# xmlyqing00/V-FloodNet

Hardware: AMD Instinct MI355X
Metric: segmented frames/sec at 480p (higher is better)
Workload: dtype f32

## Files before the change

include/vfn_hip.h:

```cpp
#ifndef VFN_HIP_H
#define VFN_HIP_H

#ifdef __cplusplus
extern "C" {
#endif

#define VFN_ABI_VERSION 15
enum { VFN_DESC_CONV = 0, VFN_DESC_STEM = 1, VFN_DESC_BANKSCAN = 2, VFN_DESC_MEMREAD = 3, VFN_DESC_BANK = 4, VFN_DESC_WGRAD = 5,
       VFN_DESC_REFRESH_FILTER = 6, VFN_DESC_REFRESH_EPILOGUE = 7, VFN_DESC_GATHER = 8, VFN_DESC_BANKMATCH = 9 };
int vfn_abi_version(void);
int vfn_sizeof_desc(int which);

typedef struct vfn_conv_desc {
    const float* in;
    const float* w;
    const float* scale;
    const float* shift;
    const float* res;
    float* out;
    int N, H, W, Cin, in_ld;
    int Ho, Wo, Cout, cout_pad, out_ld, res_ld;
    int KH, KW, stride, pad;
    int relu_in, relu_out;
    int M;
    int ksplit;
    int split_from;
    int res_mod;
    float* partial;
    int* tile_counters;
    int w_packed;
    int in_lp;
    int out_lp_relu;
    void* out_lp;
    const float* mask;
    int mask_ld;
    int mask_after;
    int w_batch_rows;
    int k_rot;
} vfn_conv_desc;

int vfn_conv_cfg_count(void);
int vfn_conv_cfg_tile(int cfg, int* bm, int* bn);
int vfn_conv_cfg_info(int cfg, int* bm, int* bn, int* wm, int* wn, int* dma);
int vfn_conv_cfg_modes(int cfg);
int vfn_conv_cfg_wk(int cfg);
int vfn_conv_cfg_tpb(int cfg);
#define VFN_CONV_SK_WS_FLOATS (16 * 1024 * 1024)
#define VFN_CONV_SK_MAX_TILES 16384
int vfn_conv_cfg_kind(int cfg);
int vfn_conv_cfg_name(int cfg, char* buf, int n);
int vfn_conv2d_nhwc_f32(const vfn_conv_desc* d, int cfg, void* stream);
int vfn_conv2d_nhwc_bf16(const vfn_conv_desc* d, int cfg, void* stream);
int vfn_conv2d_nhwc_bf16x3(const vfn_conv_desc* d, int cfg, void* stream);

int vfn_winograd_tiles(int N, int H, int W);
int vfn_winograd_input_f32(const float* x, int N, int H, int W, int C, int ld_x, int relu, float* V, int rows_pad, void* stream);
int vfn_winograd_output_f32(const float* Mb, int rows_pad, int N, int H, int W, int Cout, const float* scale, const float* shift,
                            const float* res, int res_ld, int res_mod, int relu_out, float* out, int out_ld, void* stream);
int vfn_winograd_output_masked_f32(const float* Mb, int rows_pad, int N, int H, int W, int Cout, const float* res, int res_ld,
                                   const float* mask, int mask_ld, int mask_after, float* out, int out_ld, void* stream);
int vfn_winograd_gemm_f32(const float* V, const float* U, float* Mb, int comps, int rows_pad, int C, int Cout, int cout_pad, int cfg,
                          int wgs, void* stream);
int vfn_conv1x1_persistent_f32(const vfn_conv_desc* d, int cfg, int wgs, void* stream);
int vfn_winograd_input_bf16(const float* x, int N, int H, int W, int C, int ld_x, int relu, void* V, int rows_pad, void* stream);
int vfn_winograd_gemm_bf16(const void* V, const void* U, float* Mb, int comps, int rows_pad, int C, int Cout, int cout_pad, int cfg,
                           int wgs, void* stream);
int vfn_winograd_gy_f32(const float* gy, int N, int H, int W, int C, int ld, float* Z, int rows_pad, void* stream);
int vfn_winograd_dw_f32(const float* dU, int Cout, int Cin, const float* rowscale, float* dw, int accumulate, void* stream);

typedef struct vfn_stem_desc {
    const float* frame;
    const float* mask;
    const float* w;
    const float* scale;
    const float* shift;
    float* out;
    float mean[3];
    float std[3];
    int N, cin;
    int H0, W0;
    int pad_top, pad_left;
    int Hp, Wp;
    int Ho, Wo;
} vfn_stem_desc;

int vfn_stem_conv7x7_f32(const vfn_stem_desc* d, void* stream);
int vfn_maxpool3x3s2_nhwc_f32(const float* in, float* out, int N, int H, int W, int C, void* stream);

int vfn_upsample2x_add_nhwc_f32(const float* s, const float* pm, float* out, int N, int h, int w, int C,
                                int s_bcast, void* stream);
// ... 85 lines not shown
int vfn_softmax_cols_backward_f32(const float* P, const float* dP, int B, int Q, int ld, float scale, float* dS, void* stream);
int vfn_adamw_f32(float* p, const float* g, float* m, float* v, long long n, double lr, double beta1, double beta2, double eps,
                  double weight_decay, int step, void* stream);
int vfn_colsum_f32(const float* x, int M, int C, int ld, float* partial, int nb, float* out, void* stream);
#define VFN_COLSUM_COUNTERS 64
int vfn_colsum_acc_f32(const float* x, int M, int C, int ld, float* partial, int nb, float* out, int accumulate, int* counter,
                       void* stream);
int vfn_upsample2x_add_backward_f32(const float* gm, float* gs, float* gpm, int N, int h, int w, int C, int s_bcast,
                                    void* stream);
int vfn_segment_loss_f32(const float* logit, const int* label, int bs, int obj_n, int n, float lu, float* partial, float* stats,
                         float* grad, void* stream);
int vfn_segment_uncertainty_backward_f32(const float* logit, int bs, int obj_n, int n, const float* g_unc_dev,
                                         const float* g_scores, float* partial, float* stats, float* grad, void* stream);
int vfn_tail_grad_o_f32(const float* G, const float* p_up, const float* unc, const float* conf, const float* q, float* g_o,
                        int obj_n, int h, int w, int pad_top, int pad_left, int H0, int W0, void* stream);
int vfn_tail_split_f32(const float* g_p2, const float* unc, const float* conf, const float* q, float* g_q, float* g_cf, float* g_u,
                       int obj_n, int npix, void* stream);
int vfn_local_stats_backward_f32(const float* g_lm, const float* lm, const float* g_cf, const float* g_u, const float* g_p2,
                                 const float* r1, const float* rough, const float* p_up, float* dA, float* dBv, int* amax,
                                 float* g_r1, float* g_pup, int obj_n, int h, int w, int C, void* stream);

typedef struct vfn_bankscan_desc {
    const float* q;
    const float* bank_k;
    const int* bank_len;
    const float* rowscale;
    float* part;
    long long stride_q, stride_k, stride_rs;
    float scale;
    int ldq, q_per_obj, HW, obj_n, nsplit, mode;
    int precision;
    int* work_counter;
    const void* bank_k_lp;
    float* scores;
    long long stride_scores;
} vfn_bankscan_desc;

typedef struct vfn_memread_desc {
    const float* q;
    const float* qv;
    const float* bank_k;
    const float* bank_v;
    const int* bank_len;
    const float* ml;
    float* o_part;
    int* cnt;
    float* info;
    float* out;
    long long stride_k, stride_v, stride_cnt, stride_info;
    float scale, thres;
    int ldq, ldqv, ld_out, HW, obj_n, nsplit;
    int precision;
    const void* bank_k_lp;
    const void* bank_v_lp;
    const float* scores;
    long long stride_scores;
} vfn_memread_desc;

int vfn_bank_scan(const vfn_bankscan_desc* d, void* stream);
int vfn_bank_scan_finish(const float* part, int nsplit, int HW, int obj_n, int mode, float* ml, int* idx,
                         float* corr, const float* colscale, void* stream);
int vfn_memread_apply(const vfn_memread_desc* d, void* stream);

typedef struct vfn_bankmatch_desc {
    const float* q;
    const float* bank_k;
    const void* bank_k_lp;
    const int* bank_len;
    const float* rowscale;
    const float* qnorm;
    const float* colscale;
    float* part_x3;
    float* part_f32;
    int* ulist;
    int* ucount;
    int* utotal;
    int* work_counter;
    int* match_idx;
    float* match_corr;
    long long stride_q, stride_k, stride_rs;
    int ldq, HW, obj_n;
    int nsplit;
    int nsplit_fb;
} vfn_bankmatch_desc;
int vfn_bank_match_certified(const vfn_bankmatch_desc* d, void* stream);
int vfn_memread_finish(const vfn_memread_desc* d, void* stream);

#define VFN_BANK_MAX_HW 32768
typedef struct vfn_bank_desc {
    float* bank_k;
    float* bank_v;
    float* info;
    float* scratch_k;
    float* scratch_v;
    float* scratch_info;
    const int* bank_len;
    int* bank_len_rw;
    const float* bank_knorm;
    const float* bank_vnorm;
    const int* match_idx;
    const float* match_corr;
    const float* new_k;
    const float* new_knorm;
    const float* new_vnorm;
    int* app_pos;
    int* keep_dst;
    int* plan;
    int* stats;
    long long stride_k, stride_v, stride_info, stride_n, stride_new;
    double class_budget;
    float thres_close, update_rate, new_hit_init;
    int frame_idx, ld_new, voff, HW, obj_n, cap;
    int rm_class;
    int rm_request;
} vfn_bank_desc;

int vfn_bank_refresh_lp(const vfn_bank_desc* d, void* bank_k_lp, void* bank_v_lp, int all_rows, void* stream);
int vfn_bank_refresh_lp_keys(const vfn_bank_desc* d, void* bank_k_lp, int all_rows, void* stream);

int vfn_row_norms(const float* x, long long stride_obj, int ld, int dim, const int* len_dev, int rows,
                  int obj_n, float* nrm, float* inv , long long stride_n, void* stream);
int vfn_bank_merge(const vfn_bank_desc* d, void* stream);
int vfn_bank_append(const vfn_bank_desc* d, void* stream);
int vfn_bank_remove(const vfn_bank_desc* d, void* stream);
int vfn_bank_refresh_norms(const vfn_bank_desc* d, float* bank_knorm, float* bank_kinv, float* bank_vnorm, void* stream);
int vfn_scatter_mean_f32(const float* src, long long src_s0, long long src_s1, const long long* index,
                         int S, float* out, long long out_s0, long long out_s1, int D, void* stream);
int vfn_scatter_mean_checked_f32(const float* src, long long src_s0, long long src_s1, const long long* index,
                                 long long index_s0, int S, float* out, long long out_s0, long long out_s1, int D,
                                 long long B, int* status, void* stream);

int vfn_resize_bicubic_f32(const float* in, float* out, int C, int Hi, int Wi, int Ho, int Wo, void* stream);
int vfn_resize_nearest_f32(const float* in, float* out, int C, int Hi, int Wi, int Ho, int Wo, void* stream);
int vfn_softmax_objects_f32(const float* score, float* prob, int obj_n, int n, void* stream);
int vfn_resize_argmax_u8(const float* prob, unsigned char* label, int obj_n, int Hi, int Wi, int Ho, int Wo,
                         void* stream);
int vfn_postprocess_pred_u8(const unsigned char* pred_host, int H, int W, unsigned char* out_host);
int vfn_postprocess_pred_device_u8(const unsigned char* pred, unsigned char* out, int* scratch, int H, int W,
                                   void* stream);

int vfn_to_tensor_u8(const unsigned char* src, float* dst, int H, int W, void* stream);
int vfn_overlay_u8(const float* frame, const unsigned char* mask, const unsigned char* palette, int* scratch,
                   unsigned char* out, int H, int W, double alpha, double cscale, void* stream);

int vfn_jpeg_entropy_decode(const unsigned char* data, long long size, short* coef, long long coef_cap,
                            unsigned short* qt, int* info);
int vfn_jpeg_idct_u8(const short* coef, const unsigned short* qt, unsigned char* plane, int blocks_per_row,
                     int block_rows, int pitch, void* stream);
int vfn_jpeg_to_tensor_f32(const unsigned char* y, const unsigned char* cb, const unsigned char* cr, int pitch_y,
                           int pitch_c, int W, int H, int hs, int vs, int ncomp, float* out_f32, unsigned char* out_u8,
                           void* stream);

int vfn_png_sizes(int H, int W, int bpp, long long* work_bytes, long long* out_bytes);
int vfn_png_deflate_u8(const unsigned char* raw, int H, int W, int bpp, void* work, unsigned char* out, int* stats,
                       void* stream);

int vfn_png_unfilter_sizes(int width, int height, int bpp, int* pitch, long long* work_bytes);
int vfn_png_unfilter_u8(const unsigned char* filtered, int width, int height, int bpp, void* work, unsigned char* raw,
                        int* status, void* stream);
int vfn_png_to_tensor_f32(const unsigned char* raw, int pitch, int width, int height, int color_type,
                          const unsigned char* palette, float* out, unsigned char* out_u8, void* stream);

int vfn_ln_stem_f32(const float* x, const float* w, const float* scale, const float* shift, float* out, int N, int H, int W, int Ho,
                    int Wo, int ld, int pad_before, void* stream);
int vfn_ln_dwconv_f32(const float* x, const float* w, const float* scale, const float* shift, float* out, int N, int H, int W, int C,
                      int ld_x, int ld_out, int k, int stride, int pad_before, int Ho, int Wo, int swish_in, void* stream);
// ... 20 lines not shown
```

v-floodnet_amd/_lib.py:

```python
import ctypes as C
import os

import torch

_HERE = os.path.dirname(os.path.abspath(__file__))
LIB_PATH = os.environ.get('VFN_LIB_PATH') or os.path.join(_HERE, 'libvfn_hip.so')

_lib = None

c_fp = C.c_void_p


class ConvDesc(C.Structure):
    _fields_ = [('inp', c_fp), ('w', c_fp), ('scale', c_fp), ('shift', c_fp), ('res', c_fp), ('out', c_fp),
                ('N', C.c_int), ('H', C.c_int), ('W', C.c_int), ('Cin', C.c_int), ('in_ld', C.c_int),
                ('Ho', C.c_int), ('Wo', C.c_int), ('Cout', C.c_int), ('cout_pad', C.c_int),
                ('out_ld', C.c_int), ('res_ld', C.c_int),
                ('KH', C.c_int), ('KW', C.c_int), ('stride', C.c_int), ('pad', C.c_int),
                ('relu_in', C.c_int), ('relu_out', C.c_int), ('M', C.c_int), ('ksplit', C.c_int),
                ('split_from', C.c_int), ('res_mod', C.c_int), ('partial', c_fp), ('tile_counters', c_fp),
                ('w_packed', C.c_int), ('in_lp', C.c_int), ('out_lp_relu', C.c_int), ('out_lp', c_fp), ('mask', c_fp), ('mask_ld', C.c_int), ('mask_after', C.c_int), ('w_batch_rows', C.c_int), ('k_rot', C.c_int)]


class WgradDesc(C.Structure):
    _fields_ = [('x', c_fp), ('gy', c_fp), ('rowscale', c_fp), ('dw', c_fp), ('partial', c_fp),
                ('N', C.c_int), ('H', C.c_int), ('W', C.c_int), ('Cin', C.c_int), ('ld_x', C.c_int),
                ('Ho', C.c_int), ('Wo', C.c_int), ('Cout', C.c_int), ('ld_g', C.c_int),
                ('k', C.c_int), ('stride', C.c_int), ('pad', C.c_int), ('relu', C.c_int), ('accumulate', C.c_int), ('ksplit', C.c_int),
                ('tile_counters', c_fp), ('batch', C.c_int), ('reserved', C.c_int), ('x_bstride', C.c_longlong), ('g_bstride', C.c_longlong)]


class RefreshFilter(C.Structure):
    _fields_ = [('src', c_fp), ('dst', c_fp), ('gamma', c_fp), ('var', c_fp), ('eps', C.c_float), ('kind', C.c_int),
                ('cout', C.c_int), ('cin', C.c_int), ('cin_off', C.c_int), ('cin_total', C.c_int), ('kh', C.c_int), ('kw', C.c_int),
                ('dst_ld', C.c_int), ('dst_row0', C.c_int), ('dst_col0', C.c_int), ('cout_ld', C.c_int), ('block0', C.c_int),
                ('reserved', C.c_int)]


class RefreshEpilogue(C.Structure):
    _fields_ = [('gamma', c_fp), ('beta', c_fp), ('mean', c_fp), ('var', c_fp), ('scale', c_fp), ('shift', c_fp),
                ('eps', C.c_float), ('C', C.c_int)]


class GatherEntry(C.Structure):
    _fields_ = [('src', c_fp), ('dst_offset', C.c_longlong), ('stride', C.c_longlong * 4), ('shape', C.c_int * 4), ('block0', C.c_int),
                ('reserved', C.c_int)]


class StemDesc(C.Structure):
    _fields_ = [('frame', c_fp), ('mask', c_fp), ('w', c_fp), ('scale', c_fp), ('shift', c_fp), ('out', c_fp),
                ('mean', C.c_float * 3), ('std', C.c_float * 3),
                ('N', C.c_int), ('cin', C.c_int), ('H0', C.c_int), ('W0', C.c_int),
                ('pad_top', C.c_int), ('pad_left', C.c_int), ('Hp', C.c_int), ('Wp', C.c_int),
                ('Ho', C.c_int), ('Wo', C.c_int)]


class BankScanDesc(C.Structure):
    _fields_ = [('q', c_fp), ('bank_k', c_fp), ('bank_len', c_fp), ('rowscale', c_fp), ('part', c_fp),
                ('stride_q', C.c_longlong), ('stride_k', C.c_longlong), ('stride_rs', C.c_longlong),
                ('scale', C.c_float),
                ('ldq', C.c_int), ('q_per_obj', C.c_int), ('HW', C.c_int), ('obj_n', C.c_int),
                ('nsplit', C.c_int), ('mode', C.c_int), ('precision', C.c_int), ('work_counter', c_fp), ('bank_k_lp', c_fp), ('scores', c_fp), ('stride_scores', C.c_longlong)]


class MemReadDesc(C.Structure):
    _fields_ = [('q', c_fp), ('qv', c_fp), ('bank_k', c_fp), ('bank_v', c_fp), ('bank_len', c_fp), ('ml', c_fp),
                ('o_part', c_fp), ('cnt', c_fp), ('info', c_fp), ('out', c_fp),
                ('stride_k', C.c_longlong), ('stride_v', C.c_longlong), ('stride_cnt', C.c_longlong),
                ('stride_info', C.c_longlong),
                ('scale', C.c_float), ('thres', C.c_float),
                ('ldq', C.c_int), ('ldqv', C.c_int), ('ld_out', C.c_int), ('HW', C.c_int), ('obj_n', C.c_int),
                ('nsplit', C.c_int), ('precision', C.c_int), ('bank_k_lp', c_fp), ('bank_v_lp', c_fp), ('scores', c_fp), ('stride_scores', C.c_longlong)]


class BankMatchDesc(C.Structure):
    _fields_ = [('q', c_fp), ('bank_k', c_fp), ('bank_k_lp', c_fp), ('bank_len', c_fp), ('rowscale', c_fp), ('qnorm', c_fp),
                ('colscale', c_fp), ('part_x3', c_fp), ('part_f32', c_fp), ('ulist', c_fp), ('ucount', c_fp), ('utotal', c_fp),
                ('work_counter', c_fp), ('match_idx', c_fp), ('match_corr', c_fp),
                ('stride_q', C.c_longlong), ('stride_k', C.c_longlong), ('stride_rs', C.c_longlong),
                ('ldq', C.c_int), ('HW', C.c_int), ('obj_n', C.c_int), ('nsplit', C.c_int), ('nsplit_fb', C.c_int)]


class BankDesc(C.Structure):
    _fields_ = [('bank_k', c_fp), ('bank_v', c_fp), ('info', c_fp),
                ('scratch_k', c_fp), ('scratch_v', c_fp), ('scratch_info', c_fp),
                ('bank_len', c_fp), ('bank_len_rw', c_fp), ('bank_knorm', c_fp), ('bank_vnorm', c_fp),
                ('match_idx', c_fp), ('match_corr', c_fp), ('new_k', c_fp), ('new_knorm', c_fp), ('new_vnorm', c_fp),
                ('app_pos', c_fp), ('keep_dst', c_fp), ('plan', c_fp), ('stats', c_fp),
                ('stride_k', C.c_longlong), ('stride_v', C.c_longlong), ('stride_info', C.c_longlong),
                ('stride_n', C.c_longlong), ('stride_new', C.c_longlong),
                ('class_budget', C.c_double),
                ('thres_close', C.c_float), ('update_rate', C.c_float), ('new_hit_init', C.c_float),
                ('frame_idx', C.c_int), ('ld_new', C.c_int), ('voff', C.c_int), ('HW', C.c_int),
                ('obj_n', C.c_int), ('cap', C.c_int), ('rm_class', C.c_int), ('rm_request', C.c_int)]


ABI_VERSION = 15
DESC_IDS = {0: ConvDesc, 1: StemDesc, 2: BankScanDesc, 3: MemReadDesc, 4: BankDesc, 5: WgradDesc, 6: RefreshFilter, 7: RefreshEpilogue, 8: GatherEntry, 9: BankMatchDesc}


def lib():
    global _lib
    if _lib is None:
        if not os.path.isfile(LIB_PATH):
            raise RuntimeError(
                f'{LIB_PATH} not found: build the HIP kernels first '
                '(python -c "import __graft_entry__ as g; g.build()" or make -C v-floodnet_amd/csrc)')
        L = C.CDLL(LIB_PATH)
        L.vfn_abi_version.restype = C.c_int
        if L.vfn_abi_version() != ABI_VERSION:
            raise RuntimeError(f'{LIB_PATH} has ABI version {L.vfn_abi_version()}, this package expects {ABI_VERSION} '
                               '(descriptor layouts differ): rebuild it (make -C v-floodnet_amd/csrc)')
        L.vfn_sizeof_desc.restype = C.c_int
        for which, cls in DESC_IDS.items():
            if L.vfn_sizeof_desc(which) != C.sizeof(cls):
                raise RuntimeError(f'{LIB_PATH}: sizeof({cls.__name__}) is {L.vfn_sizeof_desc(which)} in the library, '
                                   f'{C.sizeof(cls)} in this binding: rebuild it (make -C v-floodnet_amd/csrc)')
        _declare(L)
        _lib = L
    return _lib


def _declare(L):
    i, f, p = C.c_int, C.c_float, C.c_void_p
    L.vfn_abi_version.restype = i
    L.vfn_conv_cfg_count.restype = i
    L.vfn_conv_cfg_tile.argtypes = [i, C.POINTER(i), C.POINTER(i)]
    L.vfn_conv_cfg_info.argtypes = [i] + [C.POINTER(i)] * 5
    L.vfn_conv_cfg_wk.argtypes = [i]
    L.vfn_conv_cfg_wk.restype = i
    L.vfn_conv_cfg_tpb.argtypes = [i]
    L.vfn_conv_cfg_tpb.restype = i
    L.vfn_conv_cfg_modes.argtypes = [i]
    L.vfn_conv_cfg_modes.restype = i
    L.vfn_conv_cfg_kind.argtypes = [i]
    L.vfn_conv_cfg_name.argtypes = [i, C.c_char_p, i]
    L.vfn_conv_cfg_name.restype = i
    L.vfn_conv_cfg_kind.restype = i
    L.vfn_sizeof_desc.argtypes = [i]
    L.vfn_conv2d_nhwc_f32.argtypes = [C.POINTER(ConvDesc), i, p]
    L.vfn_conv2d_nhwc_bf16.argtypes = [C.POINTER(ConvDesc), i, p]
    L.vfn_conv2d_nhwc_bf16x3.argtypes = [C.POINTER(ConvDesc), i, p]
    L.vfn_stem_conv7x7_f32.argtypes = [C.POINTER(StemDesc), p]
    L.vfn_bank_scan.argtypes = [C.POINTER(BankScanDesc), p]
    L.vfn_memread_apply.argtypes = [C.POINTER(MemReadDesc), p]
    L.vfn_memread_finish.argtypes = [C.POINTER(MemReadDesc), p]
    L.vfn_bank_merge.argtypes = [C.POINTER(BankDesc), p]
    L.vfn_bank_append.argtypes = [C.POINTER(BankDesc), p]
    L.vfn_bank_remove.argtypes = [C.POINTER(BankDesc), p]
    L.vfn_bank_refresh_norms.argtypes = [C.POINTER(BankDesc), p, p, p, p]
    L.vfn_conv_wgrad_f32.argtypes = [C.POINTER(WgradDesc), p]
    L.vfn_bank_refresh_lp.argtypes = [C.POINTER(BankDesc), p, p, i, p]
    L.vfn_bank_refresh_lp_keys.argtypes = [C.POINTER(BankDesc), p, i, p]
    L.vfn_bank_match_certified.argtypes = [C.POINTER(BankMatchDesc), p]
    L.vfn_stem_wgrad_scratch_floats.argtypes = [i]
    L.vfn_stem_wgrad_scratch_floats.restype = i
    for name, args in SIGNATURES.items():
        fn = getattr(L, name)
        fn.argtypes = args
        fn.restype = i


_i, _f, _p = C.c_int, C.c_float, C.c_void_p
_ll = C.c_longlong
SIGNATURES = {
    'vfn_maxpool3x3s2_nhwc_f32': [_p, _p, _i, _i, _i, _i, _p],
    'vfn_upsample2x_add_nhwc_f32': [_p, _p, _p, _i, _i, _i, _i, _i, _p],
    'vfn_upsample2x_add_lp_nhwc_f32': [_p, _p, _p, _p, _i, _i, _i, _i, _i, _i, _p],
    'vfn_rough_uncertainty_f32': [_p, _p, _p, _p, _i, _i, _i, _p],
    'vfn_transpose_taps_f32': [_p, _i, _i, _i, _i, _i, _i, _i, _i, _i, _i, _i, _p, _p, _i, _p],
    'vfn_dilate2_f32': [_p, _p, _i, _i, _i, _i, _i, _i, _p],
    'vfn_bn_param_grads_f32': [_p, _p, _p, _p, _p, _i, _i, _p, _i, _p, _p, _p],
    'vfn_bn_param_grads_acc_f32': [_p, _p, _p, _p, _p, _i, _i, _p, _i, _p, _p, _i, _p, _p],
    'vfn_maxpool3x3s2_backward_f32': [_p, _p, _p, _i, _i, _i, _i, _p, _i, _p],
    'vfn_softmax_cols_f32': [_p, _i, _i, _i, _f, _p, _p],
    'vfn_softmax_cols_backward_f32': [_p, _p, _i, _i, _i, _f, _p, _p],
    'vfn_adamw_f32': [_p, _p, _p, _p, _ll, C.c_double, C.c_double, C.c_double, C.c_double, C.c_double, _i, _p],
    'vfn_colsum_f32': [_p, _i, _i, _i, _p, _i, _p, _p],
    'vfn_colsum_acc_f32': [_p, _i, _i, _i, _p, _i, _p, _i, _p, _p],
    'vfn_upsample2x_add_backward_f32': [_p, _p, _p, _i, _i, _i, _i, _i, _p],
# ... 125 lines not shown
```

v-floodnet_amd/csrc/memory_read.hip:

```cpp
#include "common.h"
#include "../../include/vfn_hip.h"
#include <type_traits>
#include <cstdlib>

namespace {

constexpr int DK = 128, DV = 512;
constexpr int CH = 64;

__device__ __forceinline__ int swz(int row, int chunk) { return row * DK + ((chunk ^ (row & 15)) << 2); }

__device__ __forceinline__ int swz64(int row, int chunk) { return row * CH + ((chunk ^ (row & 15)) << 2); }

__device__ __forceinline__ void chunk_load_async(float* sK, const float* src, int valid, int wave, int lane) {
#pragma unroll
    for (int j = 0; j < 8; ++j) {
        const int r = (wave * 8 + j) * 2 + (lane >> 5);
        const int pc = lane & 31;
        const int rr = min(r, valid - 1);
        const float* g = src + (size_t)rr * DK + ((pc ^ (r & 15)) << 2);
        __builtin_amdgcn_global_load_lds(g, sK + (wave * 8 + j) * 2 * DK, 16, 0, 0);
    }
}

__device__ __forceinline__ void score_tile(const float* sK, const float* sQ, int wr, int wq, int li, int lh, f32x16& acc) {
#pragma unroll
    for (int r = 0; r < 16; ++r) acc[r] = 0.f;
    const int ra = wr * 32 + li, rq = wq * 32 + li;
    f32x4 a[2], b[2];
    a[0] = *reinterpret_cast<const f32x4*>(sK + swz(ra, lh));
    b[0] = *reinterpret_cast<const f32x4*>(sQ + swz(rq, lh));
#pragma unroll
    for (int kk = 0; kk < 16; ++kk) {
        const int cur = kk & 1;
        if (kk + 1 < 16) {
            a[cur ^ 1] = *reinterpret_cast<const f32x4*>(sK + swz(ra, 2 * (kk + 1) + lh));
            b[cur ^ 1] = *reinterpret_cast<const f32x4*>(sQ + swz(rq, 2 * (kk + 1) + lh));
        }
#pragma unroll
        for (int t = 0; t < 4; ++t)
            acc = __builtin_amdgcn_mfma_f32_32x32x2f32(a[cur][t], b[cur][t], acc, 0, 0, 0);
    }
}

typedef __attribute__((ext_vector_type(2))) float f32x2;
typedef unsigned u32x4 __attribute__((ext_vector_type(4)));
typedef unsigned u32x2 __attribute__((ext_vector_type(2)));
typedef __attribute__((ext_vector_type(4))) __bf16 bf16x4;
typedef __attribute__((ext_vector_type(8))) __bf16 bf16x8;

__device__ __forceinline__ bf16x8 cvt8(const f32x4& a, const f32x4& b) {
    bf16x8 r;
#pragma unroll
    for (int e = 0; e < 4; ++e) { r[e] = (__bf16)a[e]; r[4 + e] = (__bf16)b[e]; }
    return r;
}
__device__ __forceinline__ void split8(const f32x4& a, const f32x4& b, bf16x8& h, bf16x8& l) {
#pragma unroll
    for (int e = 0; e < 4; ++e) {
        const __bf16 x = (__bf16)a[e], y = (__bf16)b[e];
        h[e] = x; h[4 + e] = y;
        l[e] = (__bf16)(a[e] - (float)x); l[4 + e] = (__bf16)(b[e] - (float)y);
    }
}
__device__ __forceinline__ int swzk(int row, int half, int chunk) { return row * 512 + half * 256 + ((chunk ^ (row & 15)) << 4); }
__device__ __forceinline__ int swzq(int row, int chunk) { return row * 256 + ((chunk ^ (row & 15)) << 4); }
__device__ __forceinline__ int swzp(int row, int chunk) { return row * 128 + ((chunk ^ ((row >> 1) & 7)) << 4); }

template <int NT, bool X3>
__device__ __forceinline__ void convert_chunk_inplace(float* sK, int tid) {
    constexpr int TPR = NT / CH;
    constexpr int F4 = 32 / TPR;
    const int r = tid / TPR, part = tid % TPR;
    f32x4 v[F4];
#pragma unroll
    for (int j = 0; j < F4; ++j) v[j] = *reinterpret_cast<const f32x4*>(sK + swz(r, part * F4 + j));
    __syncthreads();
    char* base = reinterpret_cast<char*>(sK);
#pragma unroll
    for (int j = 0; j < F4; j += 2) {
        bf16x8 h, l;
        split8(v[j], v[j + 1], h, l);
        const int chunk = (part * F4 + j) >> 1;
        *reinterpret_cast<bf16x8*>(base + swzk(r, 0, chunk)) = h;
// ... 439 lines not shown
#pragma unroll
                    for (int j = 0; j < 4; ++j) {
                        const int row = row0 + j;
                        if (row < B) {
                            const float s_ = acc[i][4 * g + j] * sc[j];
                            if (s_ > run_m) { run_m = s_; run_i = row; }
                        }
                    }
                }
        }
        if (c + 1 < c_hi) store_k(PAR ^ 1, std::integral_constant<int, PAR ^ 1>{});
        __syncthreads();
    };
    for (int c = c_lo; c < c_hi; c += 2) {
        body(std::integral_constant<int, 0>{}, c);
        if (c + 1 < c_hi) body(std::integral_constant<int, 1>{}, c + 1);
    }

    {
        const float om = __shfl_xor(run_m, 32, 64);
        if (MODE == 0) {
            const float ol = __shfl_xor(run_l, 32, 64);
            const float mn = fmaxf(run_m, om);
            float l = 0.f;
            if (mn > -INFINITY) l = run_l * expf(run_m - mn) + ol * expf(om - mn);
            run_m = mn; run_l = l;
        } else {
            const int oi = __shfl_xor(run_i, 32, 64);
            if (om > run_m || (om == run_m && oi < run_i)) { run_m = om; run_i = oi; }
        }
    }
    const int q = q0 + li;
    if (lh == 0 && q < p.HW) {
        float* dst = p.part + (((size_t)obj * p.nsplit + split) * p.HW + q) * 2;
        dst[0] = run_m;
        dst[1] = (MODE == 0) ? run_l : __int_as_float(run_i);
    }
  }
}

template <int MODE>
__global__ void bank_scan_finish_kernel(const float* __restrict__ part, int nsplit, int HW, int obj_n,
                                        float* __restrict__ ml, int* __restrict__ idx, float* __restrict__ corr,
                                        const float* __restrict__ colscale) {
    const int t = blockIdx.x * blockDim.x + threadIdx.x;
    const int i = min(t >> 3, obj_n * HW - 1), j = t & 7;
    const bool live = (t >> 3) < obj_n * HW;
    const int obj = i / HW, q = i - obj * HW;
    float m = -INFINITY, x = (MODE == 0) ? 0.f : __int_as_float(0x7fffffff);
    auto fold = [&](float om, float ox) {
        if (MODE == 0) {
            const float mn = fmaxf(m, om);
            if (mn > -INFINITY) x = x * expf(m - mn) + ox * expf(om - mn);
            m = mn;
        } else {
            const int i0 = __float_as_int(x), i1 = __float_as_int(ox);
            if (om > m || (om == m && i1 < i0)) { m = om; x = ox; }
        }
    };
    for (int s = j; s < nsplit; s += 8) {
        const float* src = part + (((size_t)obj * nsplit + s) * HW + q) * 2;
        fold(src[0], src[1]);
    }
    const int base = (threadIdx.x & 63) & ~7;
#pragma unroll
    for (int o = 1; o < 8; ++o) {
        const float om = __shfl(m, base + o, 64), ox = __shfl(x, base + o, 64);
        if (j == 0) fold(om, ox);
    }
    if (j != 0 || !live) return;
    if (MODE == 0) { ml[(size_t)i * 2] = m; ml[(size_t)i * 2 + 1] = x; }
    else { idx[i] = __float_as_int(x); corr[i] = m * colscale[i]; }
}

constexpr float MATCH_EPS_REL = 1.25e-4f;
constexpr float MATCH_EPS_ABS = 5.421010862427522e-20f;
constexpr float MATCH_QNORM_MAX = 1.152921504606846976e18f;

__global__ __launch_bounds__(64)
void bank_match_certify_kernel(const vfn_bankmatch_desc p) {
    const int lane = threadIdx.x, li = lane & 31, lh = lane >> 5;
    const int obj = blockIdx.y, q0 = blockIdx.x * 32;
    const int q = q0 + li, qc = min(q, p.HW - 1);
    float m = -INFINITY, m2 = -INFINITY;
    int bi = 0x7fffffff;
    auto fold = [&](float om, int oi, float o2) {
        if (om > m || (om == m && oi < bi)) { m2 = fmaxf(fmaxf(m, m2), o2); m = om; bi = oi; }
        else m2 = fmaxf(fmaxf(m2, om), o2);
    };
    const float* part = p.part_x3 + ((size_t)obj * p.nsplit * p.HW + qc) * 4;
#pragma unroll 4
    for (int s = lh; s < p.nsplit; s += 2) {
        const f32x4 v = *reinterpret_cast<const f32x4*>(part + (size_t)s * p.HW * 4);
        fold(v[0], __float_as_int(v[1]), v[2]);
    }
    fold(__shfl_xor(m, 32, 64), __shfl_xor(bi, 32, 64), __shfl_xor(m2, 32, 64));

    const size_t col = (size_t)obj * p.HW + qc;
    const float qn = p.qnorm[col];
    const float margin = 4.f * (MATCH_EPS_REL * qn + MATCH_EPS_ABS);
    const bool cert = q < p.HW && qn > 0.f && qn <= MATCH_QNORM_MAX && m > -INFINITY && m < INFINITY && (m - m2) > margin;

    const float* krow = p.bank_k + (size_t)obj * p.stride_k + (size_t)(cert ? bi : 0) * DK + 4 * lh;
    const float* qrow = p.q + (size_t)obj * p.stride_q + (size_t)qc * p.ldq + 4 * lh;
    f32x16 acc;
#pragma unroll
    for (int r = 0; r < 16; ++r) acc[r] = 0.f;
#pragma unroll
    for (int kk = 0; kk < 16; ++kk) {
        f32x4 a = *reinterpret_cast<const f32x4*>(krow + 8 * kk);
        const f32x4 b = *reinterpret_cast<const f32x4*>(qrow + 8 * kk);
        if (!cert) a = f32x4{0.f, 0.f, 0.f, 0.f};
#pragma unroll
        for (int t = 0; t < 4; ++t) acc = __builtin_amdgcn_mfma_f32_32x32x2f32(a[t], b[t], acc, 0, 0, 0);
    }
    const int rsel = (li & 3) + 4 * (li >> 3);
    float dot = 0.f;
#pragma unroll
    for (int r = 0; r < 16; ++r) dot = (r == rsel) ? acc[r] : dot;
    if (lh != ((li >> 2) & 1)) return;
    if (cert) {
        const float s_ = dot * p.rowscale[(size_t)obj * p.stride_rs + bi];
        p.match_idx[col] = bi;
        p.match_corr[col] = s_ * p.colscale[col];
    } else if (q < p.HW) {
        const int pos = atomicAdd(p.ucount + obj, 1);
        p.ulist[(size_t)obj * p.HW + pos] = q;
        if (p.utotal) atomicAdd(p.utotal + obj, 1);
    }
}

__global__ void bank_match_finish_listed_kernel(const float* __restrict__ part, int nsplit, int HW, int obj_n,
                                                const int* __restrict__ ulist, const int* __restrict__ ucount,
                                                int* __restrict__ idx, float* __restrict__ corr, const float* __restrict__ colscale) {
    const int t = blockIdx.x * blockDim.x + threadIdx.x;
    const int i = min(t >> 3, obj_n * HW - 1), j = t & 7;
    const int obj = i / HW, pos = i - obj * HW;
    const bool live = (t >> 3) < obj_n * HW && pos < ucount[obj];
    float m = -INFINITY, x = __int_as_float(0x7fffffff);
    auto fold = [&](float om, float ox) {
        const int i0 = __float_as_int(x), i1 = __float_as_int(ox);
        if (om > m || (om == m && i1 < i0)) { m = om; x = ox; }
    };
    if (live)
        for (int s = j; s < nsplit; s += 8) {
            const float* src = part + (((size_t)obj * nsplit + s) * HW + pos) * 2;
            fold(src[0], src[1]);
        }
    const int base = (threadIdx.x & 63) & ~7;
#pragma unroll
    for (int o = 1; o < 8; ++o) {
        const float om = __shfl(m, base + o, 64), ox = __shfl(x, base + o, 64);
        if (j == 0) fold(om, ox);
    }
    if (j != 0 || !live) return;
    const size_t c = (size_t)obj * HW + ulist[(size_t)obj * HW + pos];
    idx[c] = __float_as_int(x);
    corr[c] = m * colscale[c];
}

__device__ __forceinline__ int softmax_hits(f32x16& acc, float scale, float qm, float qinv, float thres, int nvalid, int rloc) {
    int cnt = 0;
#ifdef VFN_ABLATE_SOFTMAX
    for (int r = 0; r < 16; ++r) acc[r] *= qinv;
    return cnt;
#endif
    const float sm = -qm;
    if (nvalid >= CH) {
#pragma unroll
        for (int r = 0; r < 16; ++r) acc[r] = fast_exp(fmaf(acc[r], scale, sm)) * qinv;
    } else {
#pragma unroll
        for (int r = 0; r < 16; ++r) {
            const int rr = rloc + (r & 3) + 8 * (r >> 2);
            const float pv = fast_exp(fmaf(acc[r], scale, sm)) * qinv;
            acc[r] = rr < nvalid ? pv : 0.f;
        }
    }
#pragma unroll
    for (int r = 0; r < 16; ++r) {
        const unsigned long long hit = __ballot(acc[r] > thres);
        const int rlo = (r & 3) + 8 * (r >> 2);
        const int c_lo = __popcll(hit & 0xffffffffull), c_hi = __popcll(hit >> 32);
        asm volatile("v_writelane_b32 %0, %1, %2" : "+v"(cnt) : "s"(c_lo), "n"(rlo));
        asm volatile("v_writelane_b32 %0, %1, %2" : "+v"(cnt) : "s"(c_hi), "n"(rlo + 4));
    }
    return cnt;
}

__device__ int vfn_apply_linear_order = 0;
__device__ __forceinline__ void apply_item(const vfn_memread_desc& p, int& split, int& qt, int& obj) {
    const int qtiles = (int)gridDim.x / p.nsplit;
    if (vfn_apply_linear_order) { split = blockIdx.x % p.nsplit; qt = blockIdx.x / p.nsplit; obj = blockIdx.y; return; }
    const int total = (int)(gridDim.x * gridDim.y);
    const int id = (int)(blockIdx.y * gridDim.x + blockIdx.x);
    const int q = total >> 3, r = total & 7;
    const int xcd = id & 7, slot = id >> 3;
    const int L = (xcd < r ? xcd * (q + 1) : r * (q + 1) + (xcd - r) * q) + slot;
    const int pair = L / qtiles;
    qt = L - pair * qtiles;
    obj = pair / p.nsplit;
    split = pair - obj * p.nsplit;
}

constexpr int QTW = 128;
__device__ __forceinline__ void apply_slice(const vfn_memread_desc& p, int& split, int& qt, int& obj, int& q0, int& B) {
    apply_item(p, split, qt, obj);
// ... 1017 lines not shown
```

v-floodnet_amd/feature_bank.py:

```python
import numpy as np
import torch

from . import _lib, ops
from ._lib import ptr, stream, check, BankDesc, BankScanDesc, BankMatchDesc

DK, DV = 128, 512
MAX_SPLIT = 20
MAX_SPLIT_SCAN = 256
QT, QT_SCAN, CH = 64, 128, 64
MAX_HW = 32768


def pick_scan_slices(hw, obj_n, b_upper, target_items=1536, min_chunks=8):
    nchunks = max(1, (b_upper + CH - 1) // CH)
    qtiles = (hw + QT_SCAN - 1) // QT_SCAN
    import os
    if os.environ.get('VFN_NSPLIT_SCAN'):
        return max(1, min(int(os.environ['VFN_NSPLIT_SCAN']), nchunks, MAX_SPLIT_SCAN))
    want = max(1, target_items // (qtiles * obj_n))
    return max(1, min(want, nchunks // min_chunks if nchunks >= min_chunks else 1, MAX_SPLIT_SCAN))


def pick_fallback_slices(obj_n, b_upper, target_items=512, min_chunks=4):
    nchunks = max(1, (b_upper + CH - 1) // CH)
# ... 57 lines not shown
        _lib.lib()

    def _alloc(self, hw, n_init):
        self._require_gpu()
        dev = self.device
        o = self.obj_n
        cap = (int(max(self.class_budget, n_init)) + 2 * hw + 2 * CH + 63) // 64 * 64
        self._cap, self._hw = cap, hw
        self._kbuf = torch.empty(o, cap, DK, device=dev)
        self._vbuf = torch.empty(o, cap, DV, device=dev)
        self._ibuf = torch.zeros(o, cap, 2, device=dev)
        self._len_dev = torch.zeros(o, dtype=torch.int32, device=dev)
        self._stats = torch.zeros(o, 4, dtype=torch.int32, device=dev)
        self._knorm = torch.empty(o, cap, device=dev)
        self._vnorm = torch.empty(o, cap, device=dev)
        self._kinv = torch.empty(o, cap, device=dev)
        self._cnt = torch.zeros(o, cap, dtype=torch.int32, device=dev)
        self._keep_dst = torch.empty(o, cap, dtype=torch.int32, device=dev)
        self._plan = torch.zeros(o, 4, dtype=torch.int32, device=dev)
        self._new = torch.empty(o, hw, DK + DV, device=dev)
        self._nknorm = torch.empty(o, hw, device=dev)
        self._nvnorm = torch.empty(o, hw, device=dev)
        self._nkinv = torch.empty(o, hw, device=dev)
        self._midx = torch.empty(o, hw, dtype=torch.int32, device=dev)
        self._mcorr = torch.empty(o, hw, device=dev)
        self._app_pos = torch.empty(o, hw, dtype=torch.int32, device=dev)
        self._part = torch.empty(o, MAX_SPLIT_SCAN, hw, 2, device=dev)
        self._work = torch.zeros(4, dtype=torch.int32, device=dev)
        self._stats_pinned = torch.zeros(o, 4, dtype=torch.int32).pin_memory()
        self._scratch = None
        self._klp = self._vlp = None
        self._mbuf = None
        self._match_updates = 0
        self._norms_valid = self._lp_valid = self._kimg_valid = False

    def _ensure_scratch(self):
        if self._scratch is None:
            self._scratch = (torch.empty_like(self._kbuf), torch.empty_like(self._vbuf), torch.empty_like(self._ibuf))
        return self._scratch

    def _bank_desc(self):
        o, cap = self.obj_n, self._cap
        bd = BankDesc()
        bd.bank_k, bd.bank_v, bd.info = ptr(self._kbuf), ptr(self._vbuf), ptr(self._ibuf)
        bd.bank_len, bd.bank_len_rw = ptr(self._len_dev), ptr(self._len_dev)
        bd.stride_k, bd.stride_v, bd.stride_info, bd.stride_n = cap * DK, cap * DV, cap * 2, cap
        bd.HW, bd.obj_n, bd.cap = self._hw, o, cap
        return bd

    def lp_image(self):
        import os
        if os.environ.get('VFN_LP_IMAGE', '1') == '0' or self._kbuf is None:
            return None, None
        o, cap = self.obj_n, self._cap
        if self._klp is None:
            self._klp = torch.zeros(o * cap * DK * 2 + CH * DK * 2, dtype=torch.int16, device=self.device)
            self._lp_valid = self._kimg_valid = False
        if self._vlp is None:
            self._vlp = torch.zeros(o * cap * DV * 2 + CH * DV * 2, dtype=torch.int16, device=self.device)
            self._lp_valid = False
        if not self._lp_valid:
            bd = self._bank_desc()
            check(_lib.lib().vfn_bank_refresh_lp(_lib.C.byref(bd), ptr(self._klp), ptr(self._vlp), 1, stream()),
                  'vfn_bank_refresh_lp')
            self._lp_valid = self._kimg_valid = True
        return self._klp, self._vlp

    def key_image(self):
        if self._klp is None:
            self._klp = torch.zeros(self.obj_n * self._cap * DK * 2 + CH * DK * 2, dtype=torch.int16, device=self.device)
            self._lp_valid = self._kimg_valid = False
        if not self._kimg_valid:
            bd = self._bank_desc()
            check(_lib.lib().vfn_bank_refresh_lp_keys(_lib.C.byref(bd), ptr(self._klp), 1, stream()), 'vfn_bank_refresh_lp_keys')
            self._kimg_valid = True
        return self._klp

    def _match_buffers(self):
        if self._mbuf is None:
            o, hw, dev = self.obj_n, self._hw, self.device
            self._mbuf = dict(part_x3=torch.empty(o, MAX_SPLIT_SCAN, hw, 4, device=dev),
                              ulist=torch.empty(o, hw, dtype=torch.int32, device=dev),
                              ucount=torch.zeros(o, dtype=torch.int32, device=dev),
                              utotal=torch.zeros(o, dtype=torch.int32, device=dev))
        return self._mbuf

    def certified_match(self):
        import os
        return self.precision == 'fp32' and os.environ.get('VFN_CERTIFIED_MATCH', '1') != '0'

    def match_stats(self):
        unc = [0] * self.obj_n if self._mbuf is None else [int(x) for x in self._mbuf['utotal'].cpu()]
        return dict(updates=self._match_updates, columns=self._match_updates * self._hw, uncertain=unc)

    def _sync_len(self):
        if self._dirty:
            self._stats_pinned.copy_(self._stats, non_blocking=True)
            torch.cuda.current_stream().synchronize()
            self.absorb_stats(self._stats_pinned)
        return self._len_host

    def absorb_stats(self, stats_host, in_flight=0):
        st = stats_host.numpy()
        self._len_host = [int(st[i, 0]) for i in range(self.obj_n)]
        self._len_upper = [min(n + in_flight * self._hw, self._cap) for n in self._len_host]
        self._hist[self._n_updates - in_flight] = list(self._len_host)
        for k in [k for k in self._hist if k < self._n_updates - 2]:
            del self._hist[k]
        for i in range(self.obj_n):
            self.peak_n[i] = max(self.peak_n[i], float(st[i, 1]))
            self.replace_n[i] = float(st[i, 2])
        self._dirty = in_flight > 0
        for i in range(self.obj_n):
            if st[i, 3] < 0:
                code = int(st[i, 3])
                self._stats[i, 3] = 0
                if code == -1:
                    raise ValueError('cannot convert float NaN to integer (FeatureBank.remove: an entry born at '
                                     f'frame_idx with no hits, object {i})')
                raise OverflowError(f'cannot convert float infinity to integer (FeatureBank.remove, object {i})')

    def stats_device(self):
        return self._stats

    def len_upper(self):
        u = self._n_updates
        if u == 0 and 0 in self._hist:
            return max(self._hist[0])
        prev = self._hist.get(u - 1)
        if prev is not None:
            return min(max(prev) + self._hw, self._cap)
        return max(self._len_upper)

    @property
    def keys(self):
        if self._kbuf is None:
            return None
        n = self._sync_len()
        self._norms_valid = self._lp_valid = self._kimg_valid = False
        return [self._kbuf[i, :n[i]].t() for i in range(self.obj_n)]

    @keys.setter
    def keys(self, value):
        if value is None:
            self._kbuf = None
            return
        raise AttributeError('assign through init_bank()/append(): the bank lives in pre-allocated device slabs')

    @property
    def values(self):
        if self._vbuf is None:
            return None
        n = self._sync_len()
        self._norms_valid = self._lp_valid = self._kimg_valid = False
        return [self._vbuf[i, :n[i]].t() for i in range(self.obj_n)]

    @values.setter
    def values(self, value):
        if value is None:
            self._vbuf = None
            return
        raise AttributeError('assign through init_bank()/append(): the bank lives in pre-allocated device slabs')

    @property
    def info(self):
        if self._ibuf is None:
            return [None for _ in range(self.obj_n)]
        n = self._sync_len()
        return [self._ibuf[i, :n[i]] for i in range(self.obj_n)]

    @torch.no_grad()
    def _write_columns(self, keys, values, start, frame_idx, hit_init):
        for i in range(self.obj_n):
            n = keys[i].shape[1]
            s = start[i]
            self._kbuf[i, s:s + n].copy_(keys[i].t())
# ... 27 lines not shown
        ln = torch.empty(len(lens), dtype=torch.int32, pin_memory=True)
        for i, v in enumerate(lens):
            ln[i] = v
        self._len_dev.copy_(ln, non_blocking=True)
        self._dirty = False

    def append(self, keys, values, frame_idx=0):
        if self._kbuf is None:
            return self.init_bank(keys, values, frame_idx)
        lens = self._sync_len()
        need = max(lens[i] + keys[i].shape[1] for i in range(self.obj_n))
        if need > self._cap:
            self._grow(need)
        self._write_columns(keys, values, lens, frame_idx, 20.0)
        self._graph_kv = None
        self._norms_valid = self._lp_valid = self._kimg_valid = False
        self._set_lengths([lens[i] + int(keys[i].shape[1]) for i in range(self.obj_n)])

    def _grow(self, need):
        cap = (int(need * 1.5) + self._hw + 63) // 64 * 64
        lens = self._len_host
        for name in ('_kbuf', '_vbuf', '_ibuf', '_knorm', '_vnorm', '_kinv', '_cnt', '_keep_dst'):
            old = getattr(self, name)
            new = torch.zeros(old.shape[0], cap, *old.shape[2:], dtype=old.dtype, device=old.device)
            new[:, :self._cap] = old
            setattr(self, name, new)
        self._cap = cap
        self._scratch = None
        self._klp = self._vlp = None
        self._lp_valid = self._kimg_valid = False
        del lens

    def _stage_new(self, prev_key, prev_value):
        hw = prev_key[0].shape[1]
        k0 = prev_key[0]
        ld = DK + DV
        ok = k0.is_cuda and k0.dtype == torch.float32 and k0.stride() == (1, ld) and hw == self._hw
        if ok:
            base = k0.data_ptr()
            for i in range(self.obj_n):
                k, v = prev_key[i], prev_value[i]
                if (k.stride() != (1, ld) or v.stride() != (1, ld) or k.shape != (DK, hw) or v.shape != (DV, hw)
                        or k.data_ptr() != base + i * hw * ld * 4 or v.data_ptr() != k.data_ptr() + DK * 4):
                    ok = False
                    break
        if ok:
            return k0, ld
        for i in range(self.obj_n):
            self._new[i, :, :DK].copy_(prev_key[i].t())
            self._new[i, :, DK:].copy_(prev_value[i].t())
        return self._new, ld

    def update(self, prev_key, prev_value, frame_idx, update_rate=-1):
        self._require_gpu()
        self._graph_kv = None
        if update_rate == -1:
            update_rate = self.update_rate
        hw = prev_key[0].shape[1]
        if hw != self._hw:
            raise RuntimeError(f'feature count changed ({hw} vs {self._hw}): one bank serves one frame size')
        if hw > MAX_HW:
            raise RuntimeError(f'{hw} features per frame exceed the bank kernels\' limit of {MAX_HW} (VFN_BANK_MAX_HW)')
        L = _lib.lib()
        o, cap = self.obj_n, self._cap
        new, ld = self._stage_new(prev_key, prev_value)
        s = stream()

        if not self._norms_valid:
            ops.row_norms(self._kbuf, cap * DK, DK, DK, self._len_dev, 0, o, self._knorm, self._kinv, cap)
            ops.row_norms(self._vbuf, cap * DV, DV, DV, self._len_dev, 0, o, self._vnorm, None, cap)
        ops.row_norms(new, hw * ld, ld, DK, None, hw, o, self._nknorm, self._nkinv, hw)
        check(L.vfn_row_norms(_lib.C.c_void_p(new.data_ptr() + DK * 4), hw * ld, ld, DV, None, hw, o,
                              ptr(self._nvnorm), None, hw, s), 'vfn_row_norms')

        b_up = self.len_upper()
        nsplit = pick_scan_slices(hw, o, b_up)
        if self.certified_match():
            mb = self._match_buffers()
            md = BankMatchDesc()
            md.q, md.bank_k, md.bank_k_lp, md.bank_len = ptr(new), ptr(self._kbuf), ptr(self.key_image()), ptr(self._len_dev)
            md.rowscale, md.qnorm, md.colscale = ptr(self._kinv), ptr(self._nknorm), ptr(self._nkinv)
            md.part_x3, md.part_f32, md.ulist = ptr(mb['part_x3']), ptr(self._part), ptr(mb['ulist'])
            md.ucount, md.utotal, md.work_counter = ptr(mb['ucount']), ptr(mb['utotal']), ptr(self._work)
            md.match_idx, md.match_corr = ptr(self._midx), ptr(self._mcorr)
            md.stride_q, md.stride_k, md.stride_rs = hw * ld, cap * DK, cap
            md.ldq, md.HW, md.obj_n, md.nsplit = ld, hw, o, nsplit
            md.nsplit_fb = pick_fallback_slices(o, b_up)
            check(L.vfn_bank_match_certified(_lib.C.byref(md), s), 'vfn_bank_match_certified')
            self._match_updates += 1
        else:
            d = BankScanDesc()
            d.q, d.bank_k, d.bank_len, d.rowscale, d.part = ptr(new), ptr(self._kbuf), ptr(self._len_dev), ptr(self._kinv), ptr(self._part)
            d.stride_q, d.stride_k, d.stride_rs = hw * ld, cap * DK, cap
            d.scale = 1.0
            d.ldq, d.q_per_obj, d.HW, d.obj_n, d.nsplit, d.mode = ld, 1, hw, o, nsplit, 1
            d.precision = ops.MODES[self.precision]
            d.work_counter = ptr(self._work)
            if d.precision:
                klp, _ = self.lp_image()
                d.bank_k_lp = ptr(klp) if klp is not None else None
            check(L.vfn_bank_scan(_lib.C.byref(d), s), 'vfn_bank_scan')
            check(L.vfn_bank_scan_finish(ptr(self._part), nsplit, hw, o, 1, None, ptr(self._midx), ptr(self._mcorr),
                                         ptr(self._nkinv), s), 'vfn_bank_scan_finish')

        may_evict = self.class_budget < b_up + hw
        if may_evict:
            sk, sv, si = self._ensure_scratch()
        else:
            sk, sv, si = self._kbuf, self._vbuf, self._ibuf
        bd = BankDesc()
        bd.bank_k, bd.bank_v, bd.info = ptr(self._kbuf), ptr(self._vbuf), ptr(self._ibuf)
        bd.scratch_k, bd.scratch_v, bd.scratch_info = ptr(sk), ptr(sv), ptr(si)
        bd.bank_len, bd.bank_len_rw = ptr(self._len_dev), ptr(self._len_dev)
        bd.bank_knorm, bd.bank_vnorm = ptr(self._knorm), ptr(self._vnorm)
        bd.match_idx, bd.match_corr = ptr(self._midx), ptr(self._mcorr)
        bd.new_k, bd.new_knorm, bd.new_vnorm = ptr(new), ptr(self._nknorm), ptr(self._nvnorm)
        bd.app_pos, bd.keep_dst, bd.plan, bd.stats = ptr(self._app_pos), ptr(self._keep_dst), ptr(self._plan), ptr(self._stats)
        bd.stride_k, bd.stride_v, bd.stride_info, bd.stride_n, bd.stride_new = cap * DK, cap * DV, cap * 2, cap, hw * ld
        bd.class_budget = float(self.class_budget)
        bd.thres_close, bd.update_rate, bd.new_hit_init = float(self.thres_close), float(update_rate), 0.0
        bd.frame_idx, bd.ld_new, bd.voff, bd.HW, bd.obj_n, bd.cap = int(frame_idx), ld, DK, hw, o, cap
        bd.rm_class, bd.rm_request = -1, 0
        check(L.vfn_bank_merge(_lib.C.byref(bd), s), 'vfn_bank_merge')
        check(L.vfn_bank_append(_lib.C.byref(bd), s), 'vfn_bank_append')
        check(L.vfn_bank_refresh_norms(_lib.C.byref(bd), ptr(self._knorm), ptr(self._kinv), ptr(self._vnorm), s),
              'vfn_bank_refresh_norms')
        self._norms_valid = True
        if self._klp is not None and self._lp_valid:
            check(L.vfn_bank_refresh_lp(_lib.C.byref(bd), ptr(self._klp), ptr(self._vlp), 0, s), 'vfn_bank_refresh_lp')
        elif self._klp is not None and self._kimg_valid:
            check(L.vfn_bank_refresh_lp_keys(_lib.C.byref(bd), ptr(self._klp), 0, s), 'vfn_bank_refresh_lp_keys')

        self._dirty = True
        self._len_upper = [min(n + hw, cap) for n in self._len_upper]
        self._n_updates += 1

    def remove(self, class_idx, request_n, frame_idx):
        self._require_gpu()
        self._graph_kv = None
        L = _lib.lib()
        o, cap, hw = self.obj_n, self._cap, self._hw
        self._sync_len()
        sk, sv, si = self._ensure_scratch()
        bd = BankDesc()
        bd.bank_k, bd.bank_v, bd.info = ptr(self._kbuf), ptr(self._vbuf), ptr(self._ibuf)
        bd.scratch_k, bd.scratch_v, bd.scratch_info = ptr(sk), ptr(sv), ptr(si)
        bd.bank_len, bd.bank_len_rw = ptr(self._len_dev), ptr(self._len_dev)
        bd.match_corr = ptr(self._mcorr)
        bd.app_pos, bd.keep_dst, bd.plan, bd.stats = ptr(self._app_pos), ptr(self._keep_dst), ptr(self._plan), ptr(self._stats)
        bd.stride_k, bd.stride_v, bd.stride_info, bd.stride_n, bd.stride_new = cap * DK, cap * DV, cap * 2, cap, 0
        bd.class_budget = float(self.class_budget)
        bd.thres_close, bd.update_rate, bd.new_hit_init = float(self.thres_close), float(self.update_rate), 0.0
        bd.frame_idx, bd.ld_new, bd.voff, bd.HW, bd.obj_n, bd.cap = int(frame_idx), DK + DV, DK, hw, o, cap
        bd.rm_class, bd.rm_request = int(class_idx), int(request_n)
        check(L.vfn_bank_remove(_lib.C.byref(bd), stream()), 'vfn_bank_remove')
        self._norms_valid = self._lp_valid = self._kimg_valid = False
        self._dirty = True
        n = self._sync_len()
        return (self.class_budget - n[class_idx]) - request_n

    def state_dict(self, device='cpu'):
        if self._kbuf is None:
            raise RuntimeError('FeatureBank.state_dict: the bank is empty (init_bank first)')
        n = self._sync_len()
        dev = torch.device(device)
        take = lambda t: t.detach().to(dev, copy=True)
        return dict(version=1, obj_n=self.obj_n, hw=self._hw, dk=DK, dv=DV, class_budget=float(self.class_budget),
# ... 39 lines not shown
```

Measured before the change: 159.9.

## Certify bank matches among top-4 candidates by exact fp32 rescoring

```diff
diff --git a/include/vfn_hip.h b/include/vfn_hip.h
--- a/include/vfn_hip.h
+++ b/include/vfn_hip.h
@@ -5,7 +5,7 @@
 extern "C" {
 #endif
 
-#define VFN_ABI_VERSION 15
+#define VFN_ABI_VERSION 16
 enum { VFN_DESC_CONV = 0, VFN_DESC_STEM = 1, VFN_DESC_BANKSCAN = 2, VFN_DESC_MEMREAD = 3, VFN_DESC_BANK = 4, VFN_DESC_WGRAD = 5,
        VFN_DESC_REFRESH_FILTER = 6, VFN_DESC_REFRESH_EPILOGUE = 7, VFN_DESC_GATHER = 8, VFN_DESC_BANKMATCH = 9 };
 int vfn_abi_version(void);
@@ -257,6 +257,7 @@
     int ldq, HW, obj_n;
     int nsplit;
     int nsplit_fb;
+    int* rtotal;
 } vfn_bankmatch_desc;
 int vfn_bank_match_certified(const vfn_bankmatch_desc* d, void* stream);
 int vfn_memread_finish(const vfn_memread_desc* d, void* stream);
diff --git a/v-floodnet_amd/_lib.py b/v-floodnet_amd/_lib.py
--- a/v-floodnet_amd/_lib.py
+++ b/v-floodnet_amd/_lib.py
@@ -78,7 +78,7 @@
                 ('colscale', c_fp), ('part_x3', c_fp), ('part_f32', c_fp), ('ulist', c_fp), ('ucount', c_fp), ('utotal', c_fp),
                 ('work_counter', c_fp), ('match_idx', c_fp), ('match_corr', c_fp),
                 ('stride_q', C.c_longlong), ('stride_k', C.c_longlong), ('stride_rs', C.c_longlong),
-                ('ldq', C.c_int), ('HW', C.c_int), ('obj_n', C.c_int), ('nsplit', C.c_int), ('nsplit_fb', C.c_int)]
+                ('ldq', C.c_int), ('HW', C.c_int), ('obj_n', C.c_int), ('nsplit', C.c_int), ('nsplit_fb', C.c_int), ('rtotal', c_fp)]
 
 
 class BankDesc(C.Structure):
@@ -95,7 +95,7 @@
                 ('obj_n', C.c_int), ('cap', C.c_int), ('rm_class', C.c_int), ('rm_request', C.c_int)]
 
 
-ABI_VERSION = 15
+ABI_VERSION = 16
 DESC_IDS = {0: ConvDesc, 1: StemDesc, 2: BankScanDesc, 3: MemReadDesc, 4: BankDesc, 5: WgradDesc, 6: RefreshFilter, 7: RefreshEpilogue, 8: GatherEntry, 9: BankMatchDesc}
 
 
diff --git a/v-floodnet_amd/csrc/match_cands.h b/v-floodnet_amd/csrc/match_cands.h
--- /dev/null
+++ b/v-floodnet_amd/csrc/match_cands.h
@@ -0,0 +1,59 @@
+#pragma once
+
+#if defined(__HIPCC__)
+#define VFN_HD __host__ __device__ inline
+#else
+#define VFN_HD inline
+#endif
+
+constexpr int VFN_MATCH_CAND = 4;
+constexpr int VFN_NO_ENTRY = 0x7fffffff;
+
+VFN_HD bool vfn_match_before(float a, int i, float b, int j) { return a > b || (a == b && i < j); }
+
+struct vfn_match_cands { float v[VFN_MATCH_CAND + 1]; int i[VFN_MATCH_CAND + 1]; float m2; };
+
+VFN_HD vfn_match_cands vfn_cands_empty() {
+    vfn_match_cands c;
+    for (int k = 0; k <= VFN_MATCH_CAND; ++k) { c.v[k] = -__builtin_inff(); c.i[k] = VFN_NO_ENTRY; }
+    c.m2 = -__builtin_inff();
+    return c;
+}
+
+VFN_HD void vfn_cands_push(vfn_match_cands& c, float s, int i) {
+#if defined(__HIP_DEVICE_COMPILE__)
+#pragma unroll
+#endif
+    for (int k = 0; k <= VFN_MATCH_CAND; ++k) {
+        const bool first = vfn_match_before(s, i, c.v[k], c.i[k]);
+        const float tv = c.v[k];
+        const int ti = c.i[k];
+        c.v[k] = first ? s : tv; c.i[k] = first ? i : ti;
+        s = first ? tv : s; i = first ? ti : i;
+    }
+}
+
+VFN_HD void vfn_cands_runner_up(vfn_match_cands& c, float a2) { c.m2 = (a2 > c.m2 || a2 != a2) ? a2 : c.m2; }
+
+VFN_HD void vfn_cands_slice(vfn_match_cands& c, float a1, int i1, float a2) {
+    vfn_cands_push(c, a1, i1);
+    vfn_cands_runner_up(c, a2);
+}
+
+VFN_HD void vfn_cands_merge(vfn_match_cands& c, const vfn_match_cands& o) {
+#if defined(__HIP_DEVICE_COMPILE__)
+#pragma unroll
+#endif
+    for (int k = 0; k <= VFN_MATCH_CAND; ++k) vfn_cands_push(c, o.v[k], o.i[k]);
+    vfn_cands_runner_up(c, o.m2);
+}
+
+VFN_HD int vfn_match_settled(const vfn_match_cands& c, float margin) {
+    const float A1 = c.v[0];
+    if (!(A1 > -__builtin_inff() && A1 < __builtin_inff())) return 0;
+    if (!((A1 - c.m2) > margin)) return 0;
+    if (!((A1 - c.v[VFN_MATCH_CAND]) > margin)) return 0;
+    int n = 1;
+    for (int k = 1; k < VFN_MATCH_CAND; ++k) n += ((A1 - c.v[k]) > margin) ? 0 : 1;
+    return n;
+}
diff --git a/v-floodnet_amd/csrc/memory_read.hip b/v-floodnet_amd/csrc/memory_read.hip
--- a/v-floodnet_amd/csrc/memory_read.hip
+++ b/v-floodnet_amd/csrc/memory_read.hip
@@ -1,5 +1,6 @@
 #include "common.h"
 #include "../../include/vfn_hip.h"
+#include "match_cands.h"
 #include <type_traits>
 #include <cstdlib>
 
@@ -605,47 +606,72 @@
     const int lane = threadIdx.x, li = lane & 31, lh = lane >> 5;
     const int obj = blockIdx.y, q0 = blockIdx.x * 32;
     const int q = q0 + li, qc = min(q, p.HW - 1);
-    float m = -INFINITY, m2 = -INFINITY;
-    int bi = 0x7fffffff;
-    auto fold = [&](float om, int oi, float o2) {
-        if (om > m || (om == m && oi < bi)) { m2 = fmaxf(fmaxf(m, m2), o2); m = om; bi = oi; }
-        else m2 = fmaxf(fmaxf(m2, om), o2);
-    };
+    vfn_match_cands c = vfn_cands_empty();
     const float* part = p.part_x3 + ((size_t)obj * p.nsplit * p.HW + qc) * 4;
 #pragma unroll 4
     for (int s = lh; s < p.nsplit; s += 2) {
         const f32x4 v = *reinterpret_cast<const f32x4*>(part + (size_t)s * p.HW * 4);
-        fold(v[0], __float_as_int(v[1]), v[2]);
-    }
-    fold(__shfl_xor(m, 32, 64), __shfl_xor(bi, 32, 64), __shfl_xor(m2, 32, 64));
+        vfn_cands_slice(c, v[0], __float_as_int(v[1]), v[2]);
+    }
+    {
+        vfn_match_cands o;
+#pragma unroll
+        for (int k = 0; k <= VFN_MATCH_CAND; ++k) { o.v[k] = __shfl_xor(c.v[k], 32, 64); o.i[k] = __shfl_xor(c.i[k], 32, 64); }
+        o.m2 = __shfl_xor(c.m2, 32, 64);
+        vfn_cands_merge(c, o);
+#pragma unroll
+        for (int k = 0; k <= VFN_MATCH_CAND; ++k) { c.v[k] = __shfl(c.v[k], li, 64); c.i[k] = __shfl(c.i[k], li, 64); }
+        c.m2 = __shfl(c.m2, li, 64);
+    }
 
     const size_t col = (size_t)obj * p.HW + qc;
     const float qn = p.qnorm[col];
     const float margin = 4.f * (MATCH_EPS_REL * qn + MATCH_EPS_ABS);
-    const bool cert = q < p.HW && qn > 0.f && qn <= MATCH_QNORM_MAX && m > -INFINITY && m < INFINITY && (m - m2) > margin;
-
-    const float* krow = p.bank_k + (size_t)obj * p.stride_k + (size_t)(cert ? bi : 0) * DK + 4 * lh;
+    const int B = p.bank_len[obj];
+    int n = 0;
+    if (q < p.HW && qn > 0.f && qn <= MATCH_QNORM_MAX) n = vfn_match_settled(c, margin);
+#pragma unroll
+    for (int k = 0; k < VFN_MATCH_CAND; ++k)
+        if (k < n && (unsigned)c.i[k] >= (unsigned)B) n = 0;
+
     const float* qrow = p.q + (size_t)obj * p.stride_q + (size_t)qc * p.ldq + 4 * lh;
-    f32x16 acc;
-#pragma unroll
-    for (int r = 0; r < 16; ++r) acc[r] = 0.f;
-#pragma unroll
-    for (int kk = 0; kk < 16; ++kk) {
-        f32x4 a = *reinterpret_cast<const f32x4*>(krow + 8 * kk);
-        const f32x4 b = *reinterpret_cast<const f32x4*>(qrow + 8 * kk);
-        if (!cert) a = f32x4{0.f, 0.f, 0.f, 0.f};
-#pragma unroll
-        for (int t = 0; t < 4; ++t) acc = __builtin_amdgcn_mfma_f32_32x32x2f32(a[t], b[t], acc, 0, 0, 0);
-    }
+    f32x4 bq[16];
+#pragma unroll
+    for (int kk = 0; kk < 16; ++kk) bq[kk] = *reinterpret_cast<const f32x4*>(qrow + 8 * kk);
     const int rsel = (li & 3) + 4 * (li >> 3);
-    float dot = 0.f;
-#pragma unroll
-    for (int r = 0; r < 16; ++r) dot = (r == rsel) ? acc[r] : dot;
+    float best_f = -INFINITY;
+    int best_i = VFN_NO_ENTRY;
+    bool bad = false;
+#pragma unroll
+    for (int k = 0; k < VFN_MATCH_CAND; ++k) {
+        if (__ballot(k < n) == 0) break;
+        const bool on = k < n;
+        const int e = on ? c.i[k] : 0;
+        const float* krow = p.bank_k + (size_t)obj * p.stride_k + (size_t)e * DK + 4 * lh;
+        f32x16 acc;
+#pragma unroll
+        for (int r = 0; r < 16; ++r) acc[r] = 0.f;
+#pragma unroll
+        for (int kk = 0; kk < 16; ++kk) {
+            f32x4 a = *reinterpret_cast<const f32x4*>(krow + 8 * kk);
+            if (!on) a = f32x4{0.f, 0.f, 0.f, 0.f};
+#pragma unroll
+            for (int t = 0; t < 4; ++t) acc = __builtin_amdgcn_mfma_f32_32x32x2f32(a[t], bq[kk][t], acc, 0, 0, 0);
+        }
+        float dot = 0.f;
+#pragma unroll
+        for (int r = 0; r < 16; ++r) dot = (r == rsel) ? acc[r] : dot;
+        const float f = dot * p.rowscale[(size_t)obj * p.stride_rs + e];
+        if (on) {
+            bad |= !(f > -INFINITY && f < INFINITY);
+            if (vfn_match_before(f, e, best_f, best_i)) { best_f = f; best_i = e; }
+        }
+    }
     if (lh != ((li >> 2) & 1)) return;
-    if (cert) {
-        const float s_ = dot * p.rowscale[(size_t)obj * p.stride_rs + bi];
-        p.match_idx[col] = bi;
-        p.match_corr[col] = s_ * p.colscale[col];
+    if (n > 0 && !bad) {
+        p.match_idx[col] = best_i;
+        p.match_corr[col] = best_f * p.colscale[col];
+        if (n > 1 && p.rtotal) atomicAdd(p.rtotal + obj, 1);
     } else if (q < p.HW) {
         const int pos = atomicAdd(p.ucount + obj, 1);
         p.ulist[(size_t)obj * p.HW + pos] = q;
diff --git a/v-floodnet_amd/feature_bank.py b/v-floodnet_amd/feature_bank.py
--- a/v-floodnet_amd/feature_bank.py
+++ b/v-floodnet_amd/feature_bank.py
@@ -163,7 +163,8 @@
             self._mbuf = dict(part_x3=torch.empty(o, MAX_SPLIT_SCAN, hw, 4, device=dev),
                               ulist=torch.empty(o, hw, dtype=torch.int32, device=dev),
                               ucount=torch.zeros(o, dtype=torch.int32, device=dev),
-                              utotal=torch.zeros(o, dtype=torch.int32, device=dev))
+                              utotal=torch.zeros(o, dtype=torch.int32, device=dev),
+                              rtotal=torch.zeros(o, dtype=torch.int32, device=dev))
         return self._mbuf
 
     def certified_match(self):
@@ -172,7 +173,8 @@
 
     def match_stats(self):
         unc = [0] * self.obj_n if self._mbuf is None else [int(x) for x in self._mbuf['utotal'].cpu()]
-        return dict(updates=self._match_updates, columns=self._match_updates * self._hw, uncertain=unc)
+        res = [0] * self.obj_n if self._mbuf is None else [int(x) for x in self._mbuf['rtotal'].cpu()]
+        return dict(updates=self._match_updates, columns=self._match_updates * self._hw, uncertain=unc, rescored=res)
 
     def _sync_len(self):
         if self._dirty:
@@ -366,7 +368,7 @@
             md.rowscale, md.qnorm, md.colscale = ptr(self._kinv), ptr(self._nknorm), ptr(self._nkinv)
             md.part_x3, md.part_f32, md.ulist = ptr(mb['part_x3']), ptr(self._part), ptr(mb['ulist'])
             md.ucount, md.utotal, md.work_counter = ptr(mb['ucount']), ptr(mb['utotal']), ptr(self._work)
-            md.match_idx, md.match_corr = ptr(self._midx), ptr(self._mcorr)
+            md.match_idx, md.match_corr, md.rtotal = ptr(self._midx), ptr(self._mcorr), ptr(mb['rtotal'])
             md.stride_q, md.stride_k, md.stride_rs = hw * ld, cap * DK, cap
             md.ldq, md.HW, md.obj_n, md.nsplit = ld, hw, o, nsplit
             md.nsplit_fb = pick_fallback_slices(o, b_up)
```

Result: no change. 159.6, median of 2 (-0.2%).
